# georgeliu233/STrajNet

Hardware: AMD Instinct MI355X
Metric: scenes/sec (fwd+bwd, 256x256 grids) (higher is better)
Workload: dtype bf16; 1 GPU; STrajNet cfg-256 train step (fwd+OGMFlow_loss+bwd+Nadam), batch 8/GPU, 8 waypoints, obs+occ+flow heads, fg_msa+fg, random-init weights; global_batch=8, grid=256x256x11, parallelism=dp1, hipgraph=True, concurrent_branch_streams=True, optimizer_in_step=True, settle_steps=40

## Files before the change

include/strajnet_hip.h:

```cpp
#ifndef STRAJNET_HIP_H
#define STRAJNET_HIP_H
#include <hip/hip_runtime_api.h>
#ifdef __cplusplus
extern "C" {
#endif

enum stj_status { STJ_OK = 0, STJ_EINVAL = -1, STJ_ELAUNCH = -2, STJ_EUNSUPPORTED = -3 };
enum stj_dtype { STJ_F32 = 0, STJ_BF16 = 1, STJ_F16 = 2 };
enum stj_act { STJ_ACT_NONE = 0, STJ_ACT_GELU = 1, STJ_ACT_ELU = 2 };
enum stj_unary { STJ_U_GELU = 1, STJ_U_ELU = 2, STJ_U_TANH_SCALE = 3 };

const char* stj_last_error(void);
int stj_abi_version(void);

int stj_gemm(const void* A, const void* B, void* C, const float* bias, const void* res, float* colsum,
             int M, int N, int K, int nb1, int nb2,
             long long sAb1, long long sAb2, long long sAm, long long sAk,
             long long sBb1, long long sBb2, long long sBk, long long sBn,
             long long sCb1, long long sCb2, long long ldc,
             long long sBias1, long long sBias2, long long sRes1, long long sRes2, long long ldres,
             int act, float alpha, int dtype, int c_f32, int accumulate, int splitk,
             int nkb, long long sAkb, long long sBkb, void* group, hipStream_t stream);
long long stj_gemm_group_workspace_bytes(void);
int stj_gemm_group_begin(void* group);
int stj_gemm_group_end(void* group, hipStream_t stream);
typedef struct stj_wgrad_job {
  const void* x; const void* dy; float* dw; float* db;
  int rows, cin, cout, nb1, nb2;
  long long ldx, lddy, lddw;
  long long sx1, sx2, sdy1, sdy2, sdw1, sdw2, sdb1, sdb2;
} stj_wgrad_job;
int stj_wgrad_job_supported(const stj_wgrad_job* job, int dtype);
int stj_wgrad_group(const stj_wgrad_job* jobs, int njobs, int dtype, int wg_budget, hipStream_t stream);
int stj_colsum(const void* X, float* out, int M, int N, long long ld, int dtype, hipStream_t stream);
int stj_cast(const void* src, int sdtype, void* dst, int ddtype, long long n, hipStream_t stream);

int stj_unary_fwd(const void* x, void* y, long long n, int op, float p0, int dtype, hipStream_t stream);
int stj_unary_bwd(const void* dy, const void* saved, void* dx, long long n, int op, float p0, int dtype, hipStream_t stream);
int stj_maxpool_fwd(const void* x, void* y, int* idx, long long outer, int Tn, int C, int dtype, hipStream_t stream);
int stj_maxpool_bwd(const void* dy, const void* x, const void* y, void* dx, long long outer, int Tn, int C, int dtype, hipStream_t stream);

int stj_layernorm_fwd(const void* x, const float* gamma, const float* beta, void* y, float* mean, float* rstd,
                      long long rows, int C, float eps, int gather_res, int C0, long long group_rows, int ngroups,
                      long long gstride, int dtype, hipStream_t stream);
int stj_layernorm_res_fwd(const void* x, const float* gamma, const float* beta, const void* res, void* y, float* mean,
                          float* rstd, long long rows, int C, float eps, long long group_rows, int ngroups,
                          long long gstride, int dtype, hipStream_t stream);
int stj_layernorm_bwd(const void* dy, const void* x, const float* gamma, const float* mean, const float* rstd,
// ... 34 lines not shown
long long stj_xattn_pack_workspace_bytes(int dtype);
long long stj_xattn_pack_tail_workspace_bytes(int dtype);
int stj_xattn_pack(const float* wq, const float* wo, const float* w1, const float* w2, long long zstride, int Z, void* pack, int dtype,
                   hipStream_t stream);
int stj_xattn_fwd(const void* query, const void* k, const void* v, const int* kvalid, const void* pack, const float* bo,
                  const float* g1, const float* be1, const float* b1, const float* b2, const float* g2, const float* be2,
                  long long zstride, void* y, void* sq, void* so, void* sv1, void* su2, int Z, int B, int HW,
                  const long long* rng_state, int site_a, int site_1, int site_2, float p_drop, int dtype, hipStream_t stream);
long long stj_xattn_bwd_workspace_bytes(int Z, int B, int HW);
int stj_xattn_bwd(const void* dy, const void* query, const void* k, const void* v, const int* kvalid, const void* pack,
                  const float* g1, const float* be1, const float* b1, const float* g2, long long zstride, const void* sq,
                  const void* sv1, const void* su2, void* dquery, void* dk, void* dv, float* dkp, float* dvp, void* hd,
                  void* dpre, void* du2, void* n1, void* dv1, void* dq, float* dg1, float* dbe1, float* dbo, float* dg2,
                  float* dbe2, int Z, int B, int HW, const long long* rng_state, int site_a, int site_1, int site_2,
                  float p_drop, int dtype, hipStream_t stream);

int stj_softmax_fwd(const float* S, void* P, const int* qvalid, const int* kvalid, const float* bias,
                    long long batch, int H, int Nq, int Nk, int dtype, hipStream_t stream);
int stj_softmax_bwd(const void* P, const float* dP, void* dS, long long rows, int Nk, int dtype, hipStream_t stream);
int stj_small_attn_supported(int N, int H, int d, int dtype);
int stj_small_attn_fwd(const void* q, const void* k, const void* v, const int* qvalid, const int* kvalid, void* o, long long Bt, int N, int H,
                       int d, float scale, const long long* rng_state, int site, float p_drop, int dtype, hipStream_t stream);
int stj_small_attn_bwd(const void* q, const void* k, const void* v, const int* qvalid, const int* kvalid, const void* dO, void* dq, void* dk,
                       void* dv, long long Bt, int N, int H, int d, float scale, const long long* rng_state, int site, float p_drop, int dtype,
                       hipStream_t stream);
typedef struct stj_agent_weights {
  const float* e_wq; const float* e_wk; const float* e_wv;
  const float* e_wo;
  const float* e_ws;
  const float* i_wq; const float* i_wk; const float* i_wv;
// ... 187 lines not shown
```

strajnet_amd/csrc/wgrad_sk.hip:

```cpp
#include "common.h"
#include <stdlib.h>

namespace wsk {

constexpr int TW_ = 384;
constexpr int KU = 32;
constexpr int LDW = TW_ + 16;
constexpr int CHW = LDW / 8;
constexpr int MAXJ = 28;
template <int TN> struct Geo {
  static constexpr int TN_ = TN;
  static constexpr int NWV = TN == 96 ? 4 : 8;
  static constexpr int LDN = TN == 96 ? 112 : 240;
  static constexpr int CHN = LDN / 8;
  static constexpr int IMG_N = KU * LDN * 2;
  static constexpr int STAGE = KU * (LDN + LDW) * 2;
  static constexpr int NS = TN == 96 ? 4 : 3;
  static constexpr int SLOTS = STAGE / 1024 / NWV;
  static_assert(IMG_N % 1024 == 0 && STAGE % (1024 * NWV) == 0 && LDN % 16 == 0 && (LDN / 16) % 2 == 1 && LDN >= TN + 8, "whole DMA instructions, conflict-free stride");
};

struct Job {
  const void* nar; const void* wid; float* C; float* cs;
  long long nb1s, nb2s, wb1s, wb2s, cb1s, cb2s, sb1s, sb2s;
  int ld_nar, ld_wid, ldc;
  int n_nar, n_wid;
  int t_nar, t_wid;
  int ku;
  int nb2;
  int ustart;
};
struct Desc {
  Job job[MAXJ];
  int n0, n, total0, total1;
  int g0;
};
static_assert(sizeof(Desc) <= 4096, "kernarg segment");

struct Seg {
  const char* pn; const char* pw;
  float* C; float* cs;
  int stepn, stepw;
  int ldnb, ldwb;
  int vn, vw;
  int ldc;
  int k0, k1;
};

typedef const __attribute__((address_space(4))) Desc* KD;
struct KL { KD kd; int jb, je; };

template <bool SWAP, int TN_>
__device__ __forceinline__ Seg decode(const KL& kl, int u, int uend) {
  KD kd = kl.kd;
  int j = kl.jb;
  while (j + 1 < kl.je && u >= kd->job[j + 1].ustart) ++j;
  const int local = u - kd->job[j].ustart;
  const int ku = kd->job[j].ku, t_nar = kd->job[j].t_nar, t_wid = kd->job[j].t_wid, nb2 = kd->job[j].nb2;
  const int k = local % ku;
  int t = local / ku;
  const int tn = t % t_nar; t /= t_nar;
  const int tw = t % t_wid;
  const int z = t / t_wid;
  const long long z1 = z / nb2, z2 = z % nb2;
  Seg s;
  const int ld_nar = kd->job[j].ld_nar, ld_wid = kd->job[j].ld_wid;
  s.ldnb = ld_nar * 2; s.ldwb = ld_wid * 2;
  s.stepn = KU * s.ldnb; s.stepw = KU * s.ldwb;
  s.pn = reinterpret_cast<const char*>(kd->job[j].nar) + (z1 * kd->job[j].nb1s + z2 * kd->job[j].nb2s + tn * TN_) * 2;
  s.pw = reinterpret_cast<const char*>(kd->job[j].wid) + (z1 * kd->job[j].wb1s + z2 * kd->job[j].wb2s + tw * TW_) * 2;
  s.vn = min(TN_, kd->job[j].n_nar - tn * TN_);
  s.vw = min(TW_, kd->job[j].n_wid - tw * TW_);
  s.ldc = kd->job[j].ldc;
  float* C = kd->job[j].C + z1 * kd->job[j].cb1s + z2 * kd->job[j].cb2s;
  float* cs = kd->job[j].cs;
  if (SWAP) {
    s.C = C + (long long)tw * TW_ * s.ldc + tn * TN_;
    s.cs = (cs && tw == 0) ? cs + z1 * kd->job[j].sb1s + z2 * kd->job[j].sb2s + tn * TN_ : nullptr;
  } else {
    s.C = C + (long long)tn * TN_ * s.ldc + tw * TW_;
    s.cs = (cs && tn == 0) ? cs + z1 * kd->job[j].sb1s + z2 * kd->job[j].sb2s + tw * TW_ : nullptr;
  }
  s.k0 = k;
  s.k1 = min(ku, k + (uend - u));
  return s;
}

// ... 115 lines not shown
#pragma unroll
    for (int j = 0; j < 12; ++j) bw[j] = read_tr(aW + st + j * 32, aW + st + j * 32 + 16 * LDW * 2);
#pragma unroll
    for (int a = 0; a < FA; ++a)
#pragma unroll
      for (int b = 0; b < FB; ++b) acc[a][b] = SWAP ? Mma<T>::mma(bw[a], an[b], acc[a][b]) : Mma<T>::mma(an[a], bw[b], acc[a][b]);
    if (S.cs && cs_wave) {
#pragma unroll
      for (int j = 0; j < NCS; ++j) csum[j] = frag_sum<T>(csum[j], SWAP ? an[j] : bw[j]);
    }
    ++ck;
    if (ck == S.k1) {
      asm volatile("s_waitcnt vmcnt(0)" ::: "memory");
      landed = lu - cu - 1;
      const int ldc = S.ldc;
      const int vr = SWAP ? S.vw : S.vn, vc = SWAP ? S.vn : S.vw;
      float* Cl = S.C + (long long)(row0 + 4 * g) * ldc + col0 + p;
#pragma unroll
      for (int a = 0; a < FA; ++a)
#pragma unroll
        for (int r = 0; r < 4; ++r) {
          const bool rok = row0 + 16 * a + 4 * g + r < vr;
#pragma unroll
          for (int b = 0; b < FB; ++b)
            if (rok && col0 + 16 * b + p < vc) atomicAdd(Cl + (long long)(16 * a + r) * ldc + 16 * b, acc[a][b][r]);
        }
      if (S.cs && cs_wave) {
#pragma unroll
        for (int j = 0; j < NCS; ++j) {
          float v = csum[j];
          v += __shfl_xor(v, 16, 64); v += __shfl_xor(v, 32, 64);
// ... 18 lines not shown
  KD kd = (KD)__builtin_amdgcn_kernarg_segment_ptr();
  const int g0 = kd->g0, w = blockIdx.x;
  if (w < g0) {
    const int total = kd->total0;
    const int u0 = (int)((long long)total * w / g0), u1 = (int)((long long)total * (w + 1) / g0);
    if (u0 < u1) body<T, false, TN>(KL{kd, 0, kd->n0}, u0, u1, ring);
  } else {
    const int total = kd->total1, g1 = gridDim.x - g0, w1 = w - g0;
    const int u0 = (int)((long long)total * w1 / g1), u1 = (int)((long long)total * (w1 + 1) / g1);
    if (u0 < u1) body<T, true, TN>(KL{kd, kd->n0, kd->n}, u0, u1, ring);
  }
}

}

static bool wsk_supported(const stj_wgrad_job& j, int dtype) {
  if (!stj_is16(dtype)) return false;
  if (j.rows <= 0 || j.rows % wsk::KU || j.cin <= 0 || j.cout <= 0 || j.cin % 8 || j.cout % 8 || j.nb1 <= 0 || j.nb2 <= 0) return false;
  if (((uintptr_t)j.x | (uintptr_t)j.dy) % 16) return false;
  if (j.ldx % 8 || j.lddy % 8 || j.sx1 % 8 || j.sx2 % 8 || j.sdy1 % 8 || j.sdy2 % 8) return false;
  if (j.ldx < j.cin || j.lddy < j.cout || j.lddw < j.cout) return false;
  if (j.ldx > (1 << 24) || j.lddy > (1 << 24) || j.lddw > (1 << 24)) return false;
  return true;
}

extern "C" int stj_wgrad_job_supported(const stj_wgrad_job* job, int dtype) { return job && wsk_supported(*job, dtype) ? 1 : 0; }

extern "C" int stj_wgrad_group(const stj_wgrad_job* jobs, int njobs, int dtype, int wg_budget, hipStream_t stream) {
  if (njobs <= 0) return STJ_OK;
  if (!jobs) { stj_set_error("stj_wgrad_group: NULL jobs"); return STJ_EINVAL; }
  for (int i = 0; i < njobs; ++i)
    if (!wsk_supported(jobs[i], dtype)) { stj_set_error("stj_wgrad_group: job %d is not supported (see stj_wgrad_job_supported)", i); return STJ_EUNSUPPORTED; }
  constexpr int lds96 = wsk::Geo<96>::NS * wsk::Geo<96>::STAGE, lds192 = wsk::Geo<192>::NS * wsk::Geo<192>::STAGE;
  static PerDevice<int> ncu;
  if (!ncu) {
    int dev = 0; hipDeviceProp_t pr;
    if (hipGetDevice(&dev) != hipSuccess || hipGetDeviceProperties(&pr, dev) != hipSuccess) ncu = 256;
    else ncu = pr.multiProcessorCount > 0 ? pr.multiProcessorCount : 256;
  }
  const int budget = wg_budget > 0 ? wg_budget : (int)ncu;
  auto tiles = [](int w, int t) { return (w + t - 1) / t; };
  for (int j0 = 0; j0 < njobs; j0 += wsk::MAXJ) {
    const int n = njobs - j0 < wsk::MAXJ ? njobs - j0 : wsk::MAXJ;
    int TN = 192;
    long long units192 = 0;
    for (int i = 0; i < n; ++i) {
      const stj_wgrad_job& j = jobs[j0 + i];
// ... 8 lines not shown
    auto swapped = [&](const stj_wgrad_job& j) {
      const long long cost_ns = (long long)tiles(j.cout, wsk::TW_) * j.cin + (long long)tiles(j.cin, TN) * j.cout;
      const long long cost_sw = (long long)tiles(j.cin, wsk::TW_) * j.cout + (long long)tiles(j.cout, TN) * j.cin;
      const long long nt_ns = (long long)tiles(j.cout, wsk::TW_) * tiles(j.cin, TN), nt_sw = (long long)tiles(j.cin, wsk::TW_) * tiles(j.cout, TN);
      return cost_sw < cost_ns || (cost_sw == cost_ns && nt_sw < nt_ns);
    };
    wsk::Desc d;
    long long total[2] = {0, 0}, cost[2] = {0, 0};
    int k = 0;
    for (int pass = 0; pass < 2; ++pass) {
      if (pass == 1) d.n0 = k;
      for (int i = 0; i < n; ++i) {
        const stj_wgrad_job& j = jobs[j0 + i];
        const bool sw = swapped(j);
        if ((int)sw != pass) continue;
        wsk::Job& o = d.job[k++];
        if (sw) {
          o.nar = j.dy; o.wid = j.x; o.ld_nar = (int)j.lddy; o.ld_wid = (int)j.ldx; o.n_nar = j.cout; o.n_wid = j.cin;
          o.nb1s = j.sdy1; o.nb2s = j.sdy2; o.wb1s = j.sx1; o.wb2s = j.sx2;
        } else {
          o.nar = j.x; o.wid = j.dy; o.ld_nar = (int)j.ldx; o.ld_wid = (int)j.lddy; o.n_nar = j.cin; o.n_wid = j.cout;
          o.nb1s = j.sx1; o.nb2s = j.sx2; o.wb1s = j.sdy1; o.wb2s = j.sdy2;
        }
        o.C = j.dw; o.cs = j.db; o.ldc = (int)j.lddw;
        o.cb1s = j.sdw1; o.cb2s = j.sdw2; o.sb1s = j.sdb1; o.sb2s = j.sdb2;
        o.t_nar = tiles(o.n_nar, TN); o.t_wid = tiles(o.n_wid, wsk::TW_);
        o.ku = j.rows / wsk::KU; o.nb2 = j.nb2;
        o.ustart = (int)total[pass];
        const long long units = (long long)j.nb1 * j.nb2 * o.t_nar * o.t_wid * o.ku;
        total[pass] += units;
        cost[pass] += (long long)j.nb1 * j.nb2 * o.ku * ((long long)o.t_wid * o.n_nar + (long long)o.t_nar * o.n_wid);
        if (total[pass] > (1LL << 30)) { stj_set_error("stj_wgrad_group: too many units"); return STJ_EINVAL; }
      }
    }
    d.n = k; d.total0 = (int)total[0]; d.total1 = (int)total[1];
#ifndef STJ_WSK_MINU
#define STJ_WSK_MINU 32
#endif
    long long G = (total[0] + total[1]) / STJ_WSK_MINU;
    if (G > budget) G = budget;
    if (G < 1) G = 1;
    long long g0 = cost[0] + cost[1] > 0 ? (G * cost[0] + (cost[0] + cost[1]) / 2) / (cost[0] + cost[1]) : G;
    if (total[0] > 0 && g0 < 1) g0 = 1;
    if (total[1] > 0 && g0 > G - 1) g0 = G - 1;
    if (total[0] == 0) g0 = 0;
    if (total[1] == 0) g0 = G;
// ... 3 lines not shown
    stj_with_dtype16(dtype, [&](auto t) { typedef typename decltype(t)::type T;
      if (TN == 96) {
        if ((reserved = stj_reserve_lds<wsk::wgrad_sk_kernel<T, 96>>(lds96)))
          hipLaunchKernelGGL((wsk::wgrad_sk_kernel<T, 96>), dim3((unsigned)G), dim3(256), lds96, stream, d);
      } else {
        if ((reserved = stj_reserve_lds<wsk::wgrad_sk_kernel<T, 192>>(lds192)))
          hipLaunchKernelGGL((wsk::wgrad_sk_kernel<T, 192>), dim3((unsigned)G), dim3(512), lds192, stream, d);
      }
    });
    if (!reserved) { stj_set_error("stj_wgrad_group: cannot reserve %d bytes of LDS", TN == 96 ? lds96 : lds192); return STJ_ELAUNCH; }
    int e = stj_check_launch("stj_wgrad_group");
    if (e) return e;
  }
  return STJ_OK;
}
```

strajnet_amd/csrc/xattn_fused.hip:

```cpp
#include "common.h"
#include "rng.h"
#include "chain48.h"

namespace xat {
using namespace chain;
constexpr int CB = 384, NH = 3, HS = 42, HP = 48, O1 = 128, F1 = 512, NKEY = 64, TOK = 64;
constexpr int cmax(int a, int b) { return a > b ? a : b; }

template <typename T> struct Geo {
  static constexpr int ES = (int)sizeof(T);
  static constexpr int KSTEP = Mma<T>::KSTEP;
  static constexpr int KS = CB / KSTEP;
  static constexpr int LDQ = HP + 4;
  static constexpr int KQ = ES == 2 ? 192 : 96;
  static constexpr int NQC = CB / KQ;
  static constexpr int QCH = KQ * LDQ;
  static constexpr int LDO = O1 + (ES == 2 ? 16 : 4);
  static constexpr int OCH = HP * LDO;
  static constexpr int HC = KSTEP;
  static constexpr int NFC = F1 / HC;
  static constexpr int LD1 = HC + 4;
  static constexpr int LD2 = CB + (ES == 2 ? 16 : 4);
  static constexpr int FCH = O1 * LD1 + HC * LD2;
  static constexpr int OFF_Q = 0, OFF_O = NH * NQC * QCH, OFF_F = OFF_O + NH * OCH;
// ... 883 lines not shown
  a.zstride = zstride; a.sq = const_cast<void*>(sq); a.sv1 = const_cast<void*>(sv1); a.su2 = const_cast<void*>(su2);
  a.dquery = dquery; a.dkp = dkp; a.dvp = dvp; a.hd = hd; a.dpre = dpre; a.du2 = du2; a.n1 = n1; a.dv1 = dv1; a.dq = dq;
  a.dg1 = dg1; a.dbe1 = dbe1; a.dbo = dbo; a.dg2 = dg2; a.dbe2 = dbe2; a.Z = Z; a.B = B; a.HW = HW;
  a.rng = rng_state; a.site_a = site_a; a.site_1 = site_1; a.site_2 = site_2; a.p_drop = p_drop;
  int rc = STJ_EINVAL;
  if (!stj_with_dtype(dtype, [&](auto t) { rc = xat::launch_bwd<typename decltype(t)::type>(a, stream); })) stj_set_error("xattn: bad dtype %d", dtype);
  if (rc != STJ_OK) return rc;
  const long long zb = (long long)Z * B, n = 2 * zb * xat::NKEY * xat::NH * xat::HS;
  const int grid = (int)((n + 255) / 256 > 2048 ? 2048 : (n + 255) / 256);
  const int tiles = HW / xat::TOK;
  stj_with_dtype(dtype, [&](auto t) { typedef typename decltype(t)::type T;
    hipLaunchKernelGGL(xat::xattn_dkv_reduce_kernel<T>, dim3(grid), dim3(256), 0, stream, dkp, dvp, (T*)dk, (T*)dv, zb, tiles);
  });
  return stj_check_launch("stj_xattn_dkv_reduce");
}
```

strajnet_amd/modules.py:

```python
import math
import os
from collections import OrderedDict

import numpy as np
import torch

from . import ops
from .ops import Param, ACT_NONE, ACT_ELU


def _param_spec(cfg, hb, fg_msa, fg):
    C, ws, heads, depths = cfg['embed_dim'], cfg['window_size'], cfg['num_heads'], cfg['depths']
    sp = OrderedDict()

    def add(name, shape, init):
        assert name not in sp
        sp[name] = (tuple(shape), init)

    def dense(n, i, o, bias=True):
        add(n + '/kernel', (i, o), 'glorot')
        if bias:
            add(n + '/bias', (o,), 'zeros')

    def conv(n, kh, kw, i, o, bias=True):
# ... 170 lines not shown
            self.drop_path_rate[f'flow_layers0/blocks{j}'] = float(dpr[j])
        self._seg_onehot = {}
        self.dropctx = ops.DropCtx(self.device, seed if dropout_seed is None else dropout_seed)
        self._arena = ops._ZeroArena()
        self._arena.adopt(self._gbuf[self._goff8:])
        self._dctx = None
        self._side = ops.role_stream(self.device, 'side') if (self.device.type == 'cuda' and os.environ.get('STJ_NO_SIDE_STREAM') != '1') else None
        self._side2 = ops.role_stream(self.device, 'side2') if (self._side is not None and os.environ.get('STJ_NO_SIDE_STREAM') != '2') else None
        self._streams = (self._side, self._side2)
        self.serial = False
        self.taps = None
        self.fused_mlp = self.fused_attn = os.environ.get('STJ_FUSED_SWIN', '1') != '0'
        self.fused_attn_dims = (96, 192, 384)
        self.fused_mlp_dims = (96, 192, 384)
        self.fused_xattn = True
        self.fused_stem = True
        self.agent_override = None
        self._quantize_heads = False
        self.mid_forward_hook = None
        self.fused_fgattn = True
        self.fused_agent = True
        self.fused_agent_int = True
        self.fused_quantize = True
        self.fused_fgoff = True
        self._agent_pack = None
        self._agent_pack_event = None
        self._agent_pack_stale = True
        self._fgoff_pack = None
        self._fgoff_pack_event = None
        self._fgoff_pack_stale = True
# ... 387 lines not shown
    def _zp(self, suffix):
        return self._p('cross_attn_obs0/' + suffix)

    def _xattn_params(self):
        z = self._zp
        return {'wq': z('mha/query_kernel'), 'wo': z('mha/projection_kernel'), 'bo': z('mha/projection_bias'), 'g1': z('norm1/gamma'),
                'be1': z('norm1/beta'), 'w1': z('FFN1/kernel'), 'b1': z('FFN1/bias'), 'w2': z('FFN2/kernel'), 'b2': z('FFN2/bias'),
                'g2': z('norm2/gamma'), 'be2': z('norm2/beta')}

    def _pack_xattn(self):
        self._xattn_pack = ops.xattn_pack(self._xattn_params(), self._zstride, 8, self.dtype, out=self._xattn_pack)
        self._xattn_pack_stale = False

    def _xattn_kv(self, key):
        zs = self._zstride
        with ops.gemm_group():
            pk, pv = self._zp('mha/key_kernel'), self._zp('mha/value_kernel')
            k = ops.linear_heads_in_z(key, pk.master, pk.c, pk.grad, zs, 8, True)
            v = ops.linear_heads_in_z(key, pv.master, pv.c, pv.grad, zs, 8, True)
        return k, v

    def _cross_attention_z(self, query, key, tmask):
        Z, B, HW, Cb = query.shape
        zs = self._zstride
        hs = 128 // 3
        A = key.shape[1]

        def proj_in(x, suffix, shared):
            p0 = self._zp(suffix)
            return ops.linear_heads_in_z(x, p0.master, p0.c, p0.grad, zs, 8, shared)
        if self.fused_xattn and A == 64 and HW % 64 == 0 and Cb == 384:
            k, v = self._xattn_kv(key)
# ... 227 lines not shown
```

strajnet_amd/ops.py:

```python
import contextlib
import ctypes

import os
import threading

import torch

from . import prof
from ._lib import call as _raw_call, ENUMS as _ENUMS


def call(name, *args):
    if prof.ACTIVE is None:
        return _raw_call(name, *args)
    prof.record(name, args, lambda: _raw_call(name, *args))


GROUP_GEMMS = os.environ.get('STJ_GEMM_GROUP', '1') != '0'
WS_KERNELS = os.environ.get('STJ_NO_WS') != '1'
class _GroupState(threading.local):
    def __init__(self):
        self.h = [None, None]
        self.depth = [0]

# ... 320 lines not shown
    streams = [s for s in streams if s is not None]
    if (not streams and post is None) or not out.requires_grad:
        return out
    return _JoinAfterBackward.apply(out, streams, post)


class Param:
    __slots__ = ('name', 'shape', 'master', 'c', 'grad', 'part')

    def __init__(self, name, shape, master, c, grad):
        self.name, self.shape, self.master, self.c, self.grad = name, tuple(shape), master, c, grad
        self.part = None


def gemm(A, B, C, M, N, K, sA, sB, sC, dt, bias=None, sBias=(0, 0), res=None, sRes=(0, 0, 0), nb=(1, 1),
         act=ACT_NONE, alpha=1.0, c_f32=0, accumulate=0, splitk=1, colsum=None, kseg=(1, 0, 0), post=None):
    if (accumulate and isinstance(A, torch.Tensor) and isinstance(B, torch.Tensor) and wgrad_schedule(A.device).dense_on and splitk == 0 and c_f32
            and kseg[0] == 1 and sA[2] == 1 and sB[3] == 1 and bias is None and res is None and alpha == 1.0):
        j = WJob(A, B, C, colsum, K, M, N, sA[3], sB[2], sC[2], dt, nb=nb, sx=sA[:2], sdy=sB[:2], sdw=sC[:2], sdb=sBias)
        if j.supported():
            wgrad_schedule(A.device).push(j, post)
            return True
    _gemm_call(A, B, C, M, N, K, sA, sB, sC, dt, bias, sBias, res, sRes, nb, act, alpha, c_f32, accumulate, splitk, colsum, kseg)
    return False


def _gemm_call(A, B, C, M, N, K, sA, sB, sC, dt, bias, sBias, res, sRes, nb, act, alpha, c_f32, accumulate, splitk, colsum, kseg):
    call('stj_gemm', _p(A), _p(B), _p(C), _p(bias), _p(res), _p(colsum), M, N, K, nb[0], nb[1],
         sA[0], sA[1], sA[2], sA[3], sB[0], sB[1], sB[2], sB[3], sC[0], sC[1], sC[2],
         sBias[0], sBias[1], sRes[0], sRes[1], sRes[2], act, float(alpha), dt, c_f32, accumulate, splitk,
         kseg[0], kseg[1], kseg[2], _GROUP[0], _st())


class WJob:
    __slots__ = ('x', 'dy', 'dw', 'db', 'rows', 'cin', 'cout', 'ldx', 'lddy', 'lddw', 'nb', 'sx', 'sdy', 'sdw', 'sdb', 'dt', 'keep')

    def __init__(self, x, dy, dw, db, rows, cin, cout, ldx, lddy, lddw, dt, nb=(1, 1), sx=(0, 0), sdy=(0, 0), sdw=(0, 0), sdb=(0, 0), keep=()):
        self.x, self.dy, self.dw, self.db = x, dy, dw, db
        self.rows, self.cin, self.cout, self.ldx, self.lddy, self.lddw = rows, cin, cout, ldx, lddy, lddw
        self.nb, self.sx, self.sdy, self.sdw, self.sdb, self.dt, self.keep = nb, sx, sdy, sdw, sdb, dt, keep

    def c(self):
        from ._lib import WgradJob
        return WgradJob(_p(self.x), _p(self.dy), _p(self.dw), _p(self.db), self.rows, self.cin, self.cout, self.nb[0], self.nb[1],
                        self.ldx, self.lddy, self.lddw, self.sx[0], self.sx[1], self.sdy[0], self.sdy[1], self.sdw[0], self.sdw[1],
                        self.sdb[0], self.sdb[1])

    def supported(self):
        from ._lib import lib
        return bool(lib().stj_wgrad_job_supported(ctypes.byref(self.c()), self.dt))

    def gemm(self):
        call('stj_gemm', _p(self.x), _p(self.dy), _p(self.dw), vp(0), vp(0), _p(self.db), self.cin, self.cout, self.rows, self.nb[0], self.nb[1],
             self.sx[0], self.sx[1], 1, self.ldx, self.sdy[0], self.sdy[1], self.lddy, 1, self.sdw[0], self.sdw[1], self.lddw,
             self.sdb[0], self.sdb[1], 0, 0, 0, ACT_NONE, 1.0, self.dt, 1, 1, 0, 1, 0, 0, _GROUP[0], _st())


WG_BUDGET = 0
_WJ_LAST = [None]


def _wgrad_group_model(a):
    jobs = _WJ_LAST[0]
    fl = sum(2.0 * j.rows * j.cin * j.cout * j.nb[0] * j.nb[1] for j in jobs)
    by = 0.0
    for j in jobs:
        nb, es = j.nb[0] * j.nb[1], 2
        nx = (j.nb[0] if j.sx[0] else 1) * (j.nb[1] if j.sx[1] else 1)
        by += es * j.rows * (j.cin * nx + j.cout * nb) + 4 * j.cin * j.cout * nb
    return f'wgrad_group[{len(jobs)} jobs, {sum(j.rows * j.nb[0] * j.nb[1] for j in jobs)} rows]', 'gemm_wgrad', fl, fl, by


prof.EXTRA_MODELS['stj_wgrad_group'] = _wgrad_group_model


def wgrad_group(jobs, budget=None):
    from ._lib import WgradJob
    fast = [j for j in jobs if j.supported()]
    for j in jobs:
        if j not in fast:
            j.gemm()
    if fast:
        arr = (WgradJob * len(fast))(*[j.c() for j in fast])
        _WJ_LAST[0] = fast
        call('stj_wgrad_group', ctypes.cast(arr, vp), len(fast), fast[0].dt, WG_BUDGET if budget is None else budget, _st())


def _splitk(M_out, N_out, Kdim):
    tiles = ((M_out + 63) // 64) * ((N_out + 63) // 64)
    want = max(1, 512 // max(tiles, 1))
    return int(max(1, min(want, (Kdim + 255) // 256, 256)))


class _Linear(torch.autograd.Function):
    @staticmethod
    def forward(ctx, x, trig, wc, gw, bias, gb, act, res, fold):
        _req_cuda(x)
        K, N = wc.shape
        x2 = x.contiguous().view(-1, K)
        M = x2.shape[0]
# ... 660 lines not shown
prof.EXTRA_MODELS['stj_fg_attn_fwd'] = _fgattn_cost('fwd')
prof.EXTRA_MODELS['stj_fg_attn_bwd'] = _fgattn_cost('bwd')


def xattn_pack(ps, zstride, Z, dtype, out=None):
    from ._lib import lib
    dev = ps['wq'].master.device
    nbytes = int(lib().stj_xattn_pack_workspace_bytes(DTYPE_CODE[dtype]))
    if out is None:
        out = torch.zeros(Z * nbytes + int(lib().stj_xattn_pack_tail_workspace_bytes(DTYPE_CODE[dtype])), dtype=torch.uint8, device=dev)
    call('stj_xattn_pack', _p(ps['wq'].master), _p(ps['wo'].master), _p(ps['w1'].master), _p(ps['w2'].master), zstride, Z, _p(out),
         DTYPE_CODE[dtype], _st())
    return out


class _XAttn(torch.autograd.Function):
    @staticmethod
    def forward(ctx, query, k, v, trig, kvalid, pack, ps, zstride, drop):
        _req_cuda(query, k, v)
        query, k, v = query.contiguous(), k.contiguous(), v.contiguous()
        Z, B, HW, Cb = query.shape
        dt = _dt(query)
        y = torch.empty_like(query)
        train = any(ctx.needs_input_grad[:4])
        sq = so = sv1 = su2 = None
        if train:
            sq = torch.empty((Z, B, HW, 144), dtype=query.dtype, device=query.device)
            so = torch.empty_like(sq)
            sv1 = torch.empty((Z, B, HW, 128), dtype=query.dtype, device=query.device)
            su2 = torch.empty_like(query)
# ... 24 lines not shown
        dpre = torch.empty_like(hd)
        du2 = torch.empty((Z, R, 384), dtype=ty, device=dev)
        n1 = torch.empty((Z, R, 128), dtype=ty, device=dev)
        dv1 = torch.empty_like(n1)
        dq = torch.empty((Z, R, 144), dtype=ty, device=dev)
        p_drop, state, sites = drop if drop is not None else (0.0, None, (0, 0, 0))
        call('stj_xattn_bwd', _p(dy), _p(query), _p(k), _p(v), _p(kvalid), _p(ctx.pack), _p(ps['g1'].master), _p(ps['be1'].master),
             _p(ps['b1'].master), _p(ps['g2'].master), zs, _p(sq), _p(sv1), _p(su2), _p(dquery), _p(dk), _p(dv), _p(dkp), _p(dvp), _p(hd),
             _p(dpre), _p(du2), _p(n1), _p(dv1), _p(dq), _p(ps['g1'].grad), _p(ps['be1'].grad), _p(ps['bo'].grad), _p(ps['g2'].grad),
             _p(ps['be2'].grad), Z, B, HW, _p(state), sites[0], sites[1], sites[2], float(p_drop), dt, _st())
        with gemm_group():
            gemm(hd, du2, ps['w2'].grad, 512, 384, R, (0, R * 512, 1, 512), (0, R * 384, 384, 1), (0, zs, 384), dt, nb=(1, Z), c_f32=1,
                 accumulate=1, splitk=0, colsum=ps['b2'].grad, sBias=(0, zs))
            gemm(n1, dpre, ps['w1'].grad, 128, 512, R, (0, R * 128, 1, 128), (0, R * 512, 512, 1), (0, zs, 512), dt, nb=(1, Z), c_f32=1,
                 accumulate=1, splitk=0, colsum=ps['b1'].grad, sBias=(0, zs))
            gemm(so, dv1, ps['wo'].grad, 42, 128, R, (R * 144, 48, 1, 144), (R * 128, 0, 128, 1), (zs, 42 * 128, 128), dt, nb=(Z, 3),
                 c_f32=1, accumulate=1, splitk=0)
            gemm(query, dq, ps['wq'].grad, 384, 42, R, (R * 384, 0, 1, 384), (R * 144, 48, 144, 1), (zs, 384 * 42, 42), dt, nb=(Z, 3),
                 c_f32=1, accumulate=1, splitk=0)
        return dquery, dk, dv, None, None, None, None, None, None


def xattn(query, k, v, kvalid, pack, ps, zstride, dctx=None, names=None, p_drop=0.1):
    Z, B, HW, _ = query.shape
    drop = None
    if dctx is not None:
        sites = (dctx.site(names[0], (Z, B, 3, HW, 64), p_drop), dctx.site(names[1], (Z, B * HW, 512), p_drop),
                 dctx.site(names[2], (Z, B * HW, 384), p_drop))
        drop = (float(p_drop), dctx.snap, sites)
    return _XAttn.apply(query, k, v, _trig(ps['wq'].master), kvalid, pack, ps, zstride, drop)


def _xattn_cost(kind):
    def f(a):
        if kind == 'fwd':
            Z, B, HW, dt, train = a[18], a[19], a[20], a[26], bool(getattr(a[14], 'value', None))
        else:
            Z, B, HW, dt, train = a[30], a[31], a[32], a[38], True
        es = 4 if dt == 0 else 2
        rows = Z * B * HW
        macs = 384 * 126 + 2 * 64 * 126 + 126 * 128 + 128 * 512 + 512 * 384
        fl = 2.0 * rows * macs * (1 if kind == 'fwd' else 2)
        if kind == 'fwd':
            by = es * rows * (2 * 384 + ((144 + 144 + 128 + 384) if train else 0))
        else:
# ... 1080 lines not shown
```

Measured before the change: 1413 scenes/s.

## Fuse cross-attention key/value backward into one kernel; pad head wgrad for split-K path

Adds a fused HIP kernel that computes the key-input gradient (summed over all Z key/value projections) and the key/value weight gradients in a single launch. Before, this went through generic per-head linear backward GEMMs. The change also adds 'valid' column bounds to the wgrad split-K scheduler, so the wo/wq head weight gradients can be padded from 42 to 48 columns to qualify for the grouped wgrad path. Only the first 42 columns are written. This cuts launch count and allows a faster schedule, at the cost of more complex code and some padded compute. The fused kernel only supports Z=8 and R divisible by 64.

```diff
diff --git a/include/strajnet_hip.h b/include/strajnet_hip.h
--- a/include/strajnet_hip.h
+++ b/include/strajnet_hip.h
@@ -32,6 +32,8 @@
 } stj_wgrad_job;
 int stj_wgrad_job_supported(const stj_wgrad_job* job, int dtype);
 int stj_wgrad_group(const stj_wgrad_job* jobs, int njobs, int dtype, int wg_budget, hipStream_t stream);
+int stj_wgrad_job_supported_valid(const stj_wgrad_job* job, int cin_valid, int cout_valid, int dtype);
+int stj_wgrad_group_valid(const stj_wgrad_job* jobs, const int* valid, int njobs, int dtype, int wg_budget, hipStream_t stream);
 int stj_colsum(const void* X, float* out, int M, int N, long long ld, int dtype, hipStream_t stream);
 int stj_cast(const void* src, int sdtype, void* dst, int ddtype, long long n, hipStream_t stream);
 
@@ -96,6 +98,9 @@
                   void* dpre, void* du2, void* n1, void* dv1, void* dq, float* dg1, float* dbe1, float* dbo, float* dg2,
                   float* dbe2, int Z, int B, int HW, const long long* rng_state, int site_a, int site_1, int site_2,
                   float p_drop, int dtype, hipStream_t stream);
+int stj_xattn_kv_bwd_supported(int Z, int R, long long zstride, int dtype);
+int stj_xattn_kv_bwd(const void* dk, const void* dv, const void* key, const void* wk, const void* wv, float* gwk, float* gwv,
+                     void* dkey, long long zstride, int Z, int R, int dtype, hipStream_t stream);
 
 int stj_softmax_fwd(const float* S, void* P, const int* qvalid, const int* kvalid, const float* bias,
                     long long batch, int H, int Nq, int Nk, int dtype, hipStream_t stream);
diff --git a/strajnet_amd/csrc/wgrad_sk.hip b/strajnet_amd/csrc/wgrad_sk.hip
--- a/strajnet_amd/csrc/wgrad_sk.hip
+++ b/strajnet_amd/csrc/wgrad_sk.hip
@@ -25,7 +25,7 @@
   long long nb1s, nb2s, wb1s, wb2s, cb1s, cb2s, sb1s, sb2s;
   int ld_nar, ld_wid, ldc;
   int n_nar, n_wid;
-  int t_nar, t_wid;
+  int f_nar, f_wid;
   int ku;
   int nb2;
   int ustart;
@@ -43,6 +43,7 @@
   int stepn, stepw;
   int ldnb, ldwb;
   int vn, vw;
+  int fn, fw;
   int ldc;
   int k0, k1;
 };
@@ -56,7 +57,7 @@
   int j = kl.jb;
   while (j + 1 < kl.je && u >= kd->job[j + 1].ustart) ++j;
   const int local = u - kd->job[j].ustart;
-  const int ku = kd->job[j].ku, t_nar = kd->job[j].t_nar, t_wid = kd->job[j].t_wid, nb2 = kd->job[j].nb2;
+  const int ku = kd->job[j].ku, t_nar = (kd->job[j].n_nar + TN_ - 1) / TN_, t_wid = (kd->job[j].n_wid + TW_ - 1) / TW_, nb2 = kd->job[j].nb2;
   const int k = local % ku;
   int t = local / ku;
   const int tn = t % t_nar; t /= t_nar;
@@ -71,6 +72,8 @@
   s.pw = reinterpret_cast<const char*>(kd->job[j].wid) + (z1 * kd->job[j].wb1s + z2 * kd->job[j].wb2s + tw * TW_) * 2;
   s.vn = min(TN_, kd->job[j].n_nar - tn * TN_);
   s.vw = min(TW_, kd->job[j].n_wid - tw * TW_);
+  s.fn = max(0, min(TN_, kd->job[j].f_nar - tn * TN_));
+  s.fw = max(0, min(TW_, kd->job[j].f_wid - tw * TW_));
   s.ldc = kd->job[j].ldc;
   float* C = kd->job[j].C + z1 * kd->job[j].cb1s + z2 * kd->job[j].cb2s;
   float* cs = kd->job[j].cs;
@@ -216,7 +219,7 @@
       asm volatile("s_waitcnt vmcnt(0)" ::: "memory");
       landed = lu - cu - 1;
       const int ldc = S.ldc;
-      const int vr = SWAP ? S.vw : S.vn, vc = SWAP ? S.vn : S.vw;
+      const int vr = SWAP ? S.fw : S.fn, vc = SWAP ? S.fn : S.fw;
       float* Cl = S.C + (long long)(row0 + 4 * g) * ldc + col0 + p;
 #pragma unroll
       for (int a = 0; a < FA; ++a)
@@ -265,23 +268,27 @@
 
 }
 
-static bool wsk_supported(const stj_wgrad_job& j, int dtype) {
+static bool wsk_supported(const stj_wgrad_job& j, int dtype, int cin_valid = 0, int cout_valid = 0) {
   if (!stj_is16(dtype)) return false;
   if (j.rows <= 0 || j.rows % wsk::KU || j.cin <= 0 || j.cout <= 0 || j.cin % 8 || j.cout % 8 || j.nb1 <= 0 || j.nb2 <= 0) return false;
   if (((uintptr_t)j.x | (uintptr_t)j.dy) % 16) return false;
   if (j.ldx % 8 || j.lddy % 8 || j.sx1 % 8 || j.sx2 % 8 || j.sdy1 % 8 || j.sdy2 % 8) return false;
-  if (j.ldx < j.cin || j.lddy < j.cout || j.lddw < j.cout) return false;
+  if (cin_valid < 0 || cin_valid > j.cin || cout_valid < 0 || cout_valid > j.cout) return false;
+  if (j.ldx < j.cin || j.lddy < j.cout || j.lddw < (cout_valid ? cout_valid : j.cout)) return false;
   if (j.ldx > (1 << 24) || j.lddy > (1 << 24) || j.lddw > (1 << 24)) return false;
   return true;
 }
 
 extern "C" int stj_wgrad_job_supported(const stj_wgrad_job* job, int dtype) { return job && wsk_supported(*job, dtype) ? 1 : 0; }
-
-extern "C" int stj_wgrad_group(const stj_wgrad_job* jobs, int njobs, int dtype, int wg_budget, hipStream_t stream) {
+extern "C" int stj_wgrad_job_supported_valid(const stj_wgrad_job* job, int cin_valid, int cout_valid, int dtype) {
+  return job && wsk_supported(*job, dtype, cin_valid, cout_valid) ? 1 : 0;
+}
+
+extern "C" int stj_wgrad_group_valid(const stj_wgrad_job* jobs, const int* valid, int njobs, int dtype, int wg_budget, hipStream_t stream) {
   if (njobs <= 0) return STJ_OK;
   if (!jobs) { stj_set_error("stj_wgrad_group: NULL jobs"); return STJ_EINVAL; }
   for (int i = 0; i < njobs; ++i)
-    if (!wsk_supported(jobs[i], dtype)) { stj_set_error("stj_wgrad_group: job %d is not supported (see stj_wgrad_job_supported)", i); return STJ_EUNSUPPORTED; }
+    if (!wsk_supported(jobs[i], dtype, valid ? valid[2 * i] : 0, valid ? valid[2 * i + 1] : 0)) { stj_set_error("stj_wgrad_group: job %d is not supported (see stj_wgrad_job_supported)", i); return STJ_EUNSUPPORTED; }
   constexpr int lds96 = wsk::Geo<96>::NS * wsk::Geo<96>::STAGE, lds192 = wsk::Geo<192>::NS * wsk::Geo<192>::STAGE;
   static PerDevice<int> ncu;
   if (!ncu) {
@@ -320,22 +327,25 @@
         const stj_wgrad_job& j = jobs[j0 + i];
         const bool sw = swapped(j);
         if ((int)sw != pass) continue;
+        const int cin_v = valid && valid[2 * (j0 + i)] ? valid[2 * (j0 + i)] : j.cin, cout_v = valid && valid[2 * (j0 + i) + 1] ? valid[2 * (j0 + i) + 1] : j.cout;
         wsk::Job& o = d.job[k++];
         if (sw) {
           o.nar = j.dy; o.wid = j.x; o.ld_nar = (int)j.lddy; o.ld_wid = (int)j.ldx; o.n_nar = j.cout; o.n_wid = j.cin;
           o.nb1s = j.sdy1; o.nb2s = j.sdy2; o.wb1s = j.sx1; o.wb2s = j.sx2;
+          o.f_nar = cout_v; o.f_wid = cin_v;
         } else {
           o.nar = j.x; o.wid = j.dy; o.ld_nar = (int)j.ldx; o.ld_wid = (int)j.lddy; o.n_nar = j.cin; o.n_wid = j.cout;
           o.nb1s = j.sx1; o.nb2s = j.sx2; o.wb1s = j.sdy1; o.wb2s = j.sdy2;
+          o.f_nar = cin_v; o.f_wid = cout_v;
         }
         o.C = j.dw; o.cs = j.db; o.ldc = (int)j.lddw;
         o.cb1s = j.sdw1; o.cb2s = j.sdw2; o.sb1s = j.sdb1; o.sb2s = j.sdb2;
-        o.t_nar = tiles(o.n_nar, TN); o.t_wid = tiles(o.n_wid, wsk::TW_);
+        const int t_nar = tiles(o.n_nar, TN), t_wid = tiles(o.n_wid, wsk::TW_);
         o.ku = j.rows / wsk::KU; o.nb2 = j.nb2;
         o.ustart = (int)total[pass];
-        const long long units = (long long)j.nb1 * j.nb2 * o.t_nar * o.t_wid * o.ku;
+        const long long units = (long long)j.nb1 * j.nb2 * t_nar * t_wid * o.ku;
         total[pass] += units;
-        cost[pass] += (long long)j.nb1 * j.nb2 * o.ku * ((long long)o.t_wid * o.n_nar + (long long)o.t_nar * o.n_wid);
+        cost[pass] += (long long)j.nb1 * j.nb2 * o.ku * ((long long)t_wid * o.n_nar + (long long)t_nar * o.n_wid);
         if (total[pass] > (1LL << 30)) { stj_set_error("stj_wgrad_group: too many units"); return STJ_EINVAL; }
       }
     }
@@ -369,3 +379,7 @@
   }
   return STJ_OK;
 }
+
+extern "C" int stj_wgrad_group(const stj_wgrad_job* jobs, int njobs, int dtype, int wg_budget, hipStream_t stream) {
+  return stj_wgrad_group_valid(jobs, nullptr, njobs, dtype, wg_budget, stream);
+}
diff --git a/strajnet_amd/csrc/xattn_fused.hip b/strajnet_amd/csrc/xattn_fused.hip
--- a/strajnet_amd/csrc/xattn_fused.hip
+++ b/strajnet_amd/csrc/xattn_fused.hip
@@ -921,3 +921,196 @@
   });
   return stj_check_launch("stj_xattn_dkv_reduce");
 }
+
+namespace xkv {
+using xat::CB; using xat::NH; using xat::HS; using xat::HP;
+constexpr int ZS = 8;
+constexpr int HW3 = NH * HS;
+constexpr int TR = 32, TC = 64;
+constexpr int KC = 128;
+constexpr int RB = 64;
+constexpr int TI = 64;
+constexpr int NT = 256;
+
+struct Args {
+  const void* dk; const void* dv; const void* key; const void* wk; const void* wv;
+  float* gwk; float* gwv; void* dkey;
+  long long zstride; int Z, R;
+};
+
+template <typename T> struct G {
+  static constexpr int ES = (int)sizeof(T);
+  static constexpr int V = 16 / ES;
+  static constexpr int U = 4 / ES;
+  static constexpr int NP = ES == 2 ? 2 : 1;
+  static constexpr int LDA = NP * KC + LdsPad<T>::P;
+  static constexpr int LDT = TI + (ES == 2 ? 16 : 4);
+  static constexpr int LDD = NH * HP + (ES == 2 ? 16 : 4);
+  static constexpr int NV_D = TR * HW3 / V, NV_W = TC * HS / V;
+  static constexpr int NV_K = RB * TI / V, NV_G = RB * HW3 / V;
+  static constexpr int LDS_A = (TC + TR) * LDA * ES, LDS_B = RB * (LDT + LDD) * ES;
+  static constexpr int LDS = LDS_A > LDS_B ? LDS_A : LDS_B;
+  static_assert((TR * HW3) % V == 0 && (TC * HS) % V == 0 && (RB * HW3) % V == 0 && LDS <= 65536, "whole vectors; static LDS");
+};
+constexpr int cdiv(int a, int b) { return (a + b - 1) / b; }
+
+typedef __attribute__((ext_vector_type(4))) uint32_t u32x4;
+template <int NVT> struct Run { u32x4 v[NVT]; };
+template <int NVT> __device__ __forceinline__ void run_load(Run<NVT>& r, const void* src, int nvec, int tid) {
+#pragma unroll
+  for (int j = 0; j < NVT; ++j) {
+    const int i = tid + NT * j;
+    if (i < nvec) r.v[j] = reinterpret_cast<const u32x4*>(src)[i];
+  }
+}
+template <typename T, int NVT, typename F> __device__ __forceinline__ void run_store(const Run<NVT>& r, int nvec, int tid, F place) {
+#pragma unroll
+  for (int j = 0; j < NVT; ++j) {
+    const int i = tid + NT * j;
+    if (i < nvec) {
+      constexpr int U = G<T>::U;
+      *reinterpret_cast<uint32_t*>(place((i * 4 + 0) * U)) = r.v[j][0];
+      *reinterpret_cast<uint32_t*>(place((i * 4 + 1) * U)) = r.v[j][1];
+      *reinterpret_cast<uint32_t*>(place((i * 4 + 2) * U)) = r.v[j][2];
+      *reinterpret_cast<uint32_t*>(place((i * 4 + 3) * U)) = r.v[j][3];
+    }
+  }
+}
+
+template <typename T, int NVT, int VR> __device__ __forceinline__ void slab_load(Run<NVT>& r, const T* src, long long ld, int nvec, int tid) {
+#pragma unroll
+  for (int j = 0; j < NVT; ++j) {
+    const int i = tid + NT * j;
+    if (i < nvec) r.v[j] = *reinterpret_cast<const u32x4*>(src + (i / VR) * ld + (i % VR) * G<T>::V);
+  }
+}
+template <typename T, int NVT, int VR> __device__ __forceinline__ void slab_store(const Run<NVT>& r, T* dst, int ld, int nvec, int tid) {
+#pragma unroll
+  for (int j = 0; j < NVT; ++j) {
+    const int i = tid + NT * j;
+    if (i < nvec) *reinterpret_cast<u32x4*>(dst + (i / VR) * ld + (i % VR) * G<T>::V) = r.v[j];
+  }
+}
+
+template <typename T> __device__ __forceinline__ void dkey_tile(const Args& p, const int tile, unsigned char* smem) {
+  typedef G<T> GE;
+  constexpr int LDA = GE::LDA, NVD = cdiv(GE::NV_D, NT), NVW = cdiv(GE::NV_W, NT);
+  const int tid = threadIdx.x, lane = tid & 63, wave = tid >> 6, wm = wave >> 1, wn = wave & 1;
+  const int r0 = (tile / (CB / TC)) * TR, c0 = (tile % (CB / TC)) * TC;
+  constexpr int NP = GE::NP, PAD = KC - HW3;
+  T* Ws = reinterpret_cast<T*>(smem);
+  T* Ds = Ws + TC * LDA;
+  for (int i = tid; i < (TC + TR) * NP * PAD; i += NT)
+    stf(Ws + (i / (NP * PAD)) * LDA + (i / PAD % NP) * KC + HW3 + i % PAD, 0.f);
+  f32x4 acc[2] = {(f32x4){0.f, 0.f, 0.f, 0.f}, (f32x4){0.f, 0.f, 0.f, 0.f}};
+  Run<NVD> rd[NP]; Run<NVW> rw[NP][NH];
+  auto fetch = [&](int slab) __attribute__((always_inline)) {
+#pragma unroll
+    for (int q = 0; q < NP; ++q) {
+      const int ch = slab * NP + q, z = ch >> 1;
+      const T* d = reinterpret_cast<const T*>((ch & 1) ? p.dv : p.dk) + ((long long)z * p.R + r0) * HW3;
+      const T* w = reinterpret_cast<const T*>((ch & 1) ? p.wv : p.wk) + z * p.zstride + c0 * HS;
+      run_load(rd[q], d, GE::NV_D, tid);
+#pragma unroll
+      for (int h = 0; h < NH; ++h) run_load(rw[q][h], w + h * CB * HS, GE::NV_W, tid);
+    }
+  };
+  fetch(0);
+  const int nslab = 2 * p.Z / NP;
+#pragma unroll 1
+  for (int slab = 0; slab < nslab; ++slab) {
+    __syncthreads();
+#pragma unroll
+    for (int q = 0; q < NP; ++q) {
+      run_store<T>(rd[q], GE::NV_D, tid, [&](int e) { return Ds + (e / HW3) * LDA + q * KC + e % HW3; });
+#pragma unroll
+      for (int h = 0; h < NH; ++h) run_store<T>(rw[q][h], GE::NV_W, tid, [&](int e) { return Ws + (e / HS) * LDA + q * KC + h * HS + e % HS; });
+    }
+    __syncthreads();
+    if (slab + 1 < nslab) fetch(slab + 1);
+#pragma unroll
+    for (int k0 = 0; k0 < NP * KC; k0 += Mma<T>::KSTEP) {
+      const typename Mma<T>::Frag b = Mma<T>::load(Ds, LDA, wn * 16, k0, lane);
+#pragma unroll
+      for (int i = 0; i < 2; ++i) acc[i] = Mma<T>::mma(Mma<T>::load(Ws, LDA, wm * 32 + i * 16, k0, lane), b, acc[i]);
+    }
+  }
+  T* out = reinterpret_cast<T*>(p.dkey) + (long long)(r0 + wn * 16 + (lane & 15)) * CB + c0 + wm * 32 + (lane >> 4) * 4;
+#pragma unroll
+  for (int i = 0; i < 2; ++i) {
+    const float v[4] = {acc[i][0], acc[i][1], acc[i][2], acc[i][3]};
+    st4(out + i * 16, v);
+  }
+}
+
+template <typename T> __device__ __forceinline__ void wgrad_item(const Args& p, const int item, unsigned char* smem) {
+  typedef G<T> GE;
+  constexpr int LDT = GE::LDT, LDD = GE::LDD, NVK = cdiv(GE::NV_K, NT), NVG = cdiv(GE::NV_G, NT), VR = TI / GE::V;
+  const int tid = threadIdx.x, lane = tid & 63, wave = tid >> 6;
+  const int i0 = (item % (CB / TI)) * TI, zk = item / (CB / TI), second = zk & 1, z = zk >> 1;
+  T* Ks = reinterpret_cast<T*>(smem);
+  T* Ds = Ks + RB * LDT;
+  const T* key = reinterpret_cast<const T*>(p.key) + i0;
+  const T* dsrc = reinterpret_cast<const T*>(second ? p.dv : p.dk) + (long long)z * p.R * HW3;
+  f32x4 acc[NH * 3];
+#pragma unroll
+  for (int j = 0; j < NH * 3; ++j) acc[j] = (f32x4){0.f, 0.f, 0.f, 0.f};
+  Run<NVK> rk; Run<NVG> rg;
+  auto fetch = [&](int s) __attribute__((always_inline)) {
+    slab_load<T, NVK, VR>(rk, key + (long long)s * RB * CB, CB, GE::NV_K, tid);
+    run_load(rg, dsrc + (long long)s * RB * HW3, GE::NV_G, tid);
+  };
+  fetch(0);
+  const int ns = p.R / RB;
+#pragma unroll 1
+  for (int s = 0; s < ns; ++s) {
+    __syncthreads();
+    slab_store<T, NVK, VR>(rk, Ks, LDT, GE::NV_K, tid);
+    run_store<T>(rg, GE::NV_G, tid, [&](int e) { const int c = e % HW3, h = c / HS; return Ds + (e / HW3) * LDD + h * HP + (c - h * HS); });
+    __syncthreads();
+    if (s + 1 < ns) fetch(s + 1);
+#pragma unroll
+    for (int k0 = 0; k0 < RB; k0 += Mma<T>::KSTEP) {
+      const typename Mma<T>::Frag a = Mma<T>::load_tr(Ks, LDT, wave * 16, k0, lane);
+#pragma unroll
+      for (int j = 0; j < NH * 3; ++j) acc[j] = Mma<T>::mma(a, Mma<T>::load_tr(Ds, LDD, j * 16, k0, lane), acc[j]);
+    }
+  }
+  float* gw = (second ? p.gwv : p.gwk) + z * p.zstride + (long long)(i0 + wave * 16 + (lane >> 4) * 4) * HS;
+#pragma unroll
+  for (int j = 0; j < NH * 3; ++j) {
+    const int h = j / 3, d = (j % 3) * 16 + (lane & 15);
+    if (d < HS) {
+#pragma unroll
+      for (int r = 0; r < 4; ++r) gw[(long long)h * CB * HS + r * HS + d] += acc[j][r];
+    }
+  }
+}
+
+template <typename T> __global__ __launch_bounds__(NT) void xattn_kv_bwd_kernel(const Args p) {
+  __shared__ __attribute__((aligned(16))) unsigned char smem[G<T>::LDS];
+  const int na = (p.R / TR) * (CB / TC);
+  if ((int)blockIdx.x < na) dkey_tile<T>(p, blockIdx.x, smem);
+  else wgrad_item<T>(p, blockIdx.x - na, smem);
+}
+
+static bool supported(int Z, int R, long long zstride, int dtype) {
+  return stj_dtype_ok(dtype) && Z == ZS && R > 0 && R % RB == 0 && R <= (1 << 20) && zstride % 8 == 0;
+}
+}
+
+extern "C" int stj_xattn_kv_bwd_supported(int Z, int R, long long zstride, int dtype) { return xkv::supported(Z, R, zstride, dtype) ? 1 : 0; }
+
+extern "C" int stj_xattn_kv_bwd(const void* dk, const void* dv, const void* key, const void* wk, const void* wv, float* gwk, float* gwv,
+                                void* dkey, long long zstride, int Z, int R, int dtype, hipStream_t stream) {
+  if (!xkv::supported(Z, R, zstride, dtype)) { stj_set_error("xattn_kv_bwd: Z = %d, R = %d, zstride = %lld is not taken", Z, R, zstride); return STJ_EUNSUPPORTED; }
+  if ((((uintptr_t)dk) | ((uintptr_t)dv) | ((uintptr_t)key) | ((uintptr_t)wk) | ((uintptr_t)wv) | ((uintptr_t)gwk) | ((uintptr_t)gwv) | ((uintptr_t)dkey)) & 15) {
+    stj_set_error("xattn_kv_bwd: every operand must be 16-byte aligned"); return STJ_EINVAL;
+  }
+  xkv::Args a = {dk, dv, key, wk, wv, gwk, gwv, dkey, zstride, Z, R};
+  const unsigned grid = (unsigned)((R / xkv::TR) * (xkv::CB / xkv::TC) + Z * 2 * (xkv::CB / xkv::TI));
+  stj_with_dtype(dtype, [&](auto t) { typedef typename decltype(t)::type T;
+    hipLaunchKernelGGL(xkv::xattn_kv_bwd_kernel<T>, dim3(grid), dim3(xkv::NT), 0, stream, a);
+  });
+  return stj_check_launch("stj_xattn_kv_bwd");
+}
diff --git a/strajnet_amd/modules.py b/strajnet_amd/modules.py
--- a/strajnet_amd/modules.py
+++ b/strajnet_amd/modules.py
@@ -208,6 +208,7 @@
         self.fused_attn_dims = (96, 192, 384)
         self.fused_mlp_dims = (96, 192, 384)
         self.fused_xattn = True
+        self.fused_xattn_kv = True
         self.fused_stem = True
         self.agent_override = None
         self._quantize_heads = False
@@ -625,8 +626,10 @@
 
     def _xattn_kv(self, key):
         zs = self._zstride
+        pk, pv = self._zp('mha/key_kernel'), self._zp('mha/value_kernel')
+        if self.fused_xattn_kv and ops.xattn_kv_ok(key, pk.c, zs, 8):
+            return ops.xattn_kv(key, pk, pv, zs, 8)
         with ops.gemm_group():
-            pk, pv = self._zp('mha/key_kernel'), self._zp('mha/value_kernel')
             k = ops.linear_heads_in_z(key, pk.master, pk.c, pk.grad, zs, 8, True)
             v = ops.linear_heads_in_z(key, pv.master, pv.c, pv.grad, zs, 8, True)
         return k, v
diff --git a/strajnet_amd/ops.py b/strajnet_amd/ops.py
--- a/strajnet_amd/ops.py
+++ b/strajnet_amd/ops.py
@@ -358,14 +358,14 @@
 
 
 def gemm(A, B, C, M, N, K, sA, sB, sC, dt, bias=None, sBias=(0, 0), res=None, sRes=(0, 0, 0), nb=(1, 1),
-         act=ACT_NONE, alpha=1.0, c_f32=0, accumulate=0, splitk=1, colsum=None, kseg=(1, 0, 0), post=None):
+         act=ACT_NONE, alpha=1.0, c_f32=0, accumulate=0, splitk=1, colsum=None, kseg=(1, 0, 0), post=None, valid=(0, 0)):
     if (accumulate and isinstance(A, torch.Tensor) and isinstance(B, torch.Tensor) and wgrad_schedule(A.device).dense_on and splitk == 0 and c_f32
             and kseg[0] == 1 and sA[2] == 1 and sB[3] == 1 and bias is None and res is None and alpha == 1.0):
-        j = WJob(A, B, C, colsum, K, M, N, sA[3], sB[2], sC[2], dt, nb=nb, sx=sA[:2], sdy=sB[:2], sdw=sC[:2], sdb=sBias)
+        j = WJob(A, B, C, colsum, K, M, N, sA[3], sB[2], sC[2], dt, nb=nb, sx=sA[:2], sdy=sB[:2], sdw=sC[:2], sdb=sBias, valid=valid)
         if j.supported():
             wgrad_schedule(A.device).push(j, post)
             return True
-    _gemm_call(A, B, C, M, N, K, sA, sB, sC, dt, bias, sBias, res, sRes, nb, act, alpha, c_f32, accumulate, splitk, colsum, kseg)
+    _gemm_call(A, B, C, valid[0] or M, valid[1] or N, K, sA, sB, sC, dt, bias, sBias, res, sRes, nb, act, alpha, c_f32, accumulate, splitk, colsum, kseg)
     return False
 
 
@@ -377,10 +377,12 @@
 
 
 class WJob:
-    __slots__ = ('x', 'dy', 'dw', 'db', 'rows', 'cin', 'cout', 'ldx', 'lddy', 'lddw', 'nb', 'sx', 'sdy', 'sdw', 'sdb', 'dt', 'keep')
-
-    def __init__(self, x, dy, dw, db, rows, cin, cout, ldx, lddy, lddw, dt, nb=(1, 1), sx=(0, 0), sdy=(0, 0), sdw=(0, 0), sdb=(0, 0), keep=()):
+    __slots__ = ('x', 'dy', 'dw', 'db', 'rows', 'cin', 'cout', 'ldx', 'lddy', 'lddw', 'nb', 'sx', 'sdy', 'sdw', 'sdb', 'dt', 'keep', 'valid')
+
+    def __init__(self, x, dy, dw, db, rows, cin, cout, ldx, lddy, lddw, dt, nb=(1, 1), sx=(0, 0), sdy=(0, 0), sdw=(0, 0), sdb=(0, 0), keep=(),
+                 valid=(0, 0)):
         self.x, self.dy, self.dw, self.db = x, dy, dw, db
+        self.valid = tuple(valid)
         self.rows, self.cin, self.cout, self.ldx, self.lddy, self.lddw = rows, cin, cout, ldx, lddy, lddw
         self.nb, self.sx, self.sdy, self.sdw, self.sdb, self.dt, self.keep = nb, sx, sdy, sdw, sdb, dt, keep
 
@@ -392,10 +394,10 @@
 
     def supported(self):
         from ._lib import lib
-        return bool(lib().stj_wgrad_job_supported(ctypes.byref(self.c()), self.dt))
+        return bool(lib().stj_wgrad_job_supported_valid(ctypes.byref(self.c()), self.valid[0], self.valid[1], self.dt))
 
     def gemm(self):
-        call('stj_gemm', _p(self.x), _p(self.dy), _p(self.dw), vp(0), vp(0), _p(self.db), self.cin, self.cout, self.rows, self.nb[0], self.nb[1],
+        call('stj_gemm', _p(self.x), _p(self.dy), _p(self.dw), vp(0), vp(0), _p(self.db), self.valid[0] or self.cin, self.valid[1] or self.cout, self.rows, self.nb[0], self.nb[1],
              self.sx[0], self.sx[1], 1, self.ldx, self.sdy[0], self.sdy[1], self.lddy, 1, self.sdw[0], self.sdw[1], self.lddw,
              self.sdb[0], self.sdb[1], 0, 0, 0, ACT_NONE, 1.0, self.dt, 1, 1, 0, 1, 0, 0, _GROUP[0], _st())
 
@@ -415,7 +417,7 @@
     return f'wgrad_group[{len(jobs)} jobs, {sum(j.rows * j.nb[0] * j.nb[1] for j in jobs)} rows]', 'gemm_wgrad', fl, fl, by
 
 
-prof.EXTRA_MODELS['stj_wgrad_group'] = _wgrad_group_model
+prof.EXTRA_MODELS['stj_wgrad_group'] = prof.EXTRA_MODELS['stj_wgrad_group_valid'] = _wgrad_group_model
 
 
 def wgrad_group(jobs, budget=None):
@@ -427,7 +429,11 @@
     if fast:
         arr = (WgradJob * len(fast))(*[j.c() for j in fast])
         _WJ_LAST[0] = fast
-        call('stj_wgrad_group', ctypes.cast(arr, vp), len(fast), fast[0].dt, WG_BUDGET if budget is None else budget, _st())
+        if any(j.valid != (0, 0) for j in fast):
+            val = (ctypes.c_int * (2 * len(fast)))(*[w for j in fast for w in j.valid])
+            call('stj_wgrad_group_valid', ctypes.cast(arr, vp), ctypes.cast(val, vp), len(fast), fast[0].dt, WG_BUDGET if budget is None else budget, _st())
+        else:
+            call('stj_wgrad_group', ctypes.cast(arr, vp), len(fast), fast[0].dt, WG_BUDGET if budget is None else budget, _st())
 
 
 def _splitk(M_out, N_out, Kdim):
@@ -1118,6 +1124,9 @@
     return out
 
 
+XATTN_HEAD_WGRAD_SK = True
+
+
 class _XAttn(torch.autograd.Function):
     @staticmethod
     def forward(ctx, query, k, v, trig, kvalid, pack, ps, zstride, drop):
@@ -1172,10 +1181,11 @@
                  accumulate=1, splitk=0, colsum=ps['b2'].grad, sBias=(0, zs))
             gemm(n1, dpre, ps['w1'].grad, 128, 512, R, (0, R * 128, 1, 128), (0, R * 512, 512, 1), (0, zs, 512), dt, nb=(1, Z), c_f32=1,
                  accumulate=1, splitk=0, colsum=ps['b1'].grad, sBias=(0, zs))
-            gemm(so, dv1, ps['wo'].grad, 42, 128, R, (R * 144, 48, 1, 144), (R * 128, 0, 128, 1), (zs, 42 * 128, 128), dt, nb=(Z, 3),
-                 c_f32=1, accumulate=1, splitk=0)
-            gemm(query, dq, ps['wq'].grad, 384, 42, R, (R * 384, 0, 1, 384), (R * 144, 48, 144, 1), (zs, 384 * 42, 42), dt, nb=(Z, 3),
-                 c_f32=1, accumulate=1, splitk=0)
+            hp, vo, vq = (48, (42, 0), (0, 42)) if XATTN_HEAD_WGRAD_SK else (42, (0, 0), (0, 0))
+            gemm(so, dv1, ps['wo'].grad, hp, 128, R, (R * 144, 48, 1, 144), (R * 128, 0, 128, 1), (zs, 42 * 128, 128), dt, nb=(Z, 3),
+                 c_f32=1, accumulate=1, splitk=0, valid=vo)
+            gemm(query, dq, ps['wq'].grad, 384, hp, R, (R * 384, 0, 1, 384), (R * 144, 48, 144, 1), (zs, 384 * 42, 42), dt, nb=(Z, 3),
+                 c_f32=1, accumulate=1, splitk=0, valid=vq)
         return dquery, dk, dv, None, None, None, None, None, None
 
 
@@ -1187,6 +1197,56 @@
                  dctx.site(names[2], (Z, B * HW, 384), p_drop))
         drop = (float(p_drop), dctx.snap, sites)
     return _XAttn.apply(query, k, v, _trig(ps['wq'].master), kvalid, pack, ps, zstride, drop)
+
+
+class _XAttnKV(torch.autograd.Function):
+    @staticmethod
+    def forward(ctx, key, trig, wk, gwk, wv, gwv, zstride, Z):
+        _req_cuda(key)
+        H, I, hs = wk.shape
+        x = key.contiguous()
+        R = x.numel() // I
+        dt = _dt(x)
+        k = torch.empty((Z, R, H * hs), dtype=x.dtype, device=x.device)
+        v = torch.empty_like(k)
+        with gemm_group():
+            for w0, y in ((wk, k), (wv, v)):
+                gemm(x, w0, y, R, hs, I, (0, 0, I, 1), (zstride, I * hs, hs, 1), (R * H * hs, hs, H * hs), dt, nb=(Z, H))
+        ctx.w, ctx.dims = (wk, gwk, wv, gwv), (zstride, Z, R, key.shape)
+        ctx.save_for_backward(x)
+        return k, v
+
+    @staticmethod
+    def backward(ctx, dk, dv):
+        (x,) = ctx.saved_tensors
+        wk, gwk, wv, gwv = ctx.w
+        zstride, Z, R, kshape = ctx.dims
+        dkey = torch.empty(kshape, dtype=x.dtype, device=x.device)
+        call('stj_xattn_kv_bwd', _p(dk.contiguous()), _p(dv.contiguous()), _p(x), _p(wk), _p(wv), _p(gwk), _p(gwv), _p(dkey), zstride, Z, R,
+             _dt(x), _st())
+        return (dkey,) + (None,) * 7
+
+
+def xattn_kv_ok(key, wk, zstride, Z):
+    from ._lib import lib
+    return (tuple(wk.shape) == (3, 384, 42) and key.shape[-1] == 384 and
+            bool(lib().stj_xattn_kv_bwd_supported(Z, key.numel() // 384, zstride, DTYPE_CODE[key.dtype])))
+
+
+def xattn_kv(key, pk, pv, zstride, Z):
+    return _XAttnKV.apply(key, pk.master, pk.c, pk.grad, pv.c, pv.grad, zstride, Z)
+
+
+def _xattn_kv_bwd_cost(a):
+    Z, R, dt = a[9], a[10], a[11]
+    es = 4 if dt == 0 else 2
+    nw = 2 * Z * 3 * 384 * 42
+    fl = 2 * 2.0 * R * 384 * 126 * 2 * Z
+    by = es * (2 * Z * R * 126 + 2 * R * 384 + nw) + 8 * nw
+    return f'xattn_kv_bwd[Z{Z} R{R}]', 'xattn_kv_bwd', fl, fl, by
+
+
+prof.EXTRA_MODELS['stj_xattn_kv_bwd'] = _xattn_kv_bwd_cost
 
 
 def _xattn_cost(kind):
```

New measurement: 1426 scenes/s (median of 6 runs). About the same (+0.9%).
